# halajun/VDO_SLAM

Hardware: AMD Instinct MI355X
Metric: frames/sec (per-frame hot path, KITTI-0000-shaped 1242x375) + ms/LM-iter (batch factor graph) (higher is better)
Workload: dtype f64 (LM, RANSAC) / u8,i32,f32 (front-end, tracking)

## Files before the change

### __graft_entry__.py

```python
import os
import subprocess
import sys

ROOT = os.path.dirname(os.path.abspath(__file__))
if ROOT not in sys.path:
    sys.path.insert(0, ROOT)


def build() -> None:
    env = dict(os.environ)
    jobs = str(max(1, min(16, os.cpu_count() or 2)))
    subprocess.run(["make", "-C", os.path.join(ROOT, "vdo_slam_amd", "csrc"), "-j", jobs], check=True, env=env)
    subprocess.run(["make", "-C", os.path.join(ROOT, "vdo_slam_amd", "host")], check=True, env=env)
    subprocess.run(["make", "-C", os.path.join(ROOT, "oracle"), "-j", jobs], check=True, env=env)
    from tests import oracle_lib as _ol
    _ol.load_product_epnp()
    subprocess.run(["/opt/rocm/bin/hipcc", "--offload-arch=gfx950", "-O3", "-std=c++17", "-ffp-contract=off", "-Wno-unused-value",
                    os.path.join(ROOT, "tools", "lm_dev_check.hip"), "-o", os.path.join(ROOT, "tools", "lm_dev_check")], check=True, env=env)
    subprocess.run(["/opt/rocm/bin/hipcc", "--offload-arch=gfx950", "-O3", "-std=c++17", "-ffp-contract=off", "-munsafe-fp-atomics", "-Wno-unused-value",
                    os.path.join(ROOT, "tools", "dense_check.hip"), "-o", os.path.join(ROOT, "tools", "dense_check")], check=True, env=env)
    _ol.load_ref_orb()
    _ol.load_ref_track()
    _ol.load_ref_full()
    import vdo_slam_amd
    from vdo_slam_amd import _capi
    import ctypes
    lib = ctypes.CDLL(_capi.LIB_PATH)
    assert lib.vdo_version() >= 1


def smoke() -> None:
    import ctypes as C
    import numpy as np
    from vdo_slam_amd import _capi as K, synth
    from vdo_slam_amd.ba import BatchBA, Context
    from tests import oracle_lib

    g = synth.make_ba_graph(n_frames=10, n_static=400, n_objects=2, dyn_tracks_per_object=40, seed=7)
    ctx = Context(0)
    ba = BatchBA(ctx, g)
    ba.linearize()
    S = ba.system()
    o = oracle_lib.load()
    gc, keep = K.graph_to_c(g)
    R = K.BASystem(g)
    o.vdo_oracle_ba_linearize(C.byref(gc), C.byref(R.c))
    for name in ("Hpp", "bp", "Hll", "bl", "Hpl_eb", "Hll_et", "Hlp1_et", "Hlp2_et", "Hpp_ep"):
        a, b = getattr(S, name), getattr(R, name)
        scale = max(1e-300, np.abs(b).max())
        assert np.abs(a - b).max() <= 1e-10 * scale, f"smoke: block {name} differs from oracle"
    assert abs(S.robust_chi2 - R.robust_chi2) <= 1e-10 * abs(R.robust_chi2)
    st = ba.optimize(max_iterations=5, gain_threshold=1e-4)
    assert st.iterations >= 1 and st.final_chi2 <= st.initial_chi2
    from tests import frontend_ref as R2
    from tests.test_oracle_flow2 import run_oracle
    from vdo_slam_amd import synth_frames as SF
    from vdo_slam_amd.flow2 import Flow2Batch
    from vdo_slam_amd.frontend import ORBextractor
    prob = synth.make_flow2_problem(600, seed=3)
    b = Flow2Batch(ctx, [prob]); b.run(); r = b.fetch()[0]
    T_o, _, inl_o, ninl_o, st_o = run_oracle(o, prob)
    assert r["iterations"] == st_o.iterations and r["n_inliers"] == ninl_o and np.array_equal(r["inliers"], inl_o), "smoke: flow2 LM differs from oracle"
    assert np.abs(r["T"] - T_o).max() < 1e-8
    gray = SF.make_gray(11, 640, 200)
    kp = ORBextractor(ctx, 640, 200)(gray, descriptors=True)
    ref = R2.extract_desc(o, gray)
    assert np.array_equal(kp["x"], ref["x"]) and np.array_equal(kp["y"], ref["y"]) and np.array_equal(kp["octave"], ref["octave"]), "smoke: ORB keypoints differ from oracle"
    assert np.array_equal(kp["desc"], ref["desc"]), "smoke: rotated-BRIEF descriptor bits differ from oracle"
    ba.set_estimates(g.pose, g.point)
    st3 = ba.optimize(max_iterations=5, gain_threshold=1e-4, solver=3)
    assert (st3.iterations, st3.total_trials) == (st.iterations, st.total_trials) and abs(st3.final_chi2 - st.final_chi2) <= 1e-9 * st.final_chi2, "smoke: dense MFMA solve differs from PCG"
# ... 25 lines not shown
```

### vdo_slam_amd/csrc/flow2.hip

```cpp
#include <algorithm>
#include <cmath>
#include <cstdlib>
#include <cstring>
#include <type_traits>
#include <vector>

#include "../../include/vdo_slam_hip.h"
#include "ctx.hpp"
#include "lm_dev.hpp"

namespace vdo {

struct Flow2Dev {
  int n, max_iterations, ref_quirks, pad;
  int64_t off;
  int64_t out_off, out_total;
  double K[4], Twl[16], T0[16];
  double info_flow, info_prior, huber_delta, huber_dsqr, chi2_gate;
};

struct Flow2Arrays {
  const double* in;
  double* om;
  double *Xw, *f0, *f1, *err, *B2a, *B2b, *hla, *hlb, *bla, *blb, *xl;
// ... 64 lines not shown
  template <bool TRIAL> __device__ __forceinline__ void after_exchange(double hb) {
    const double h = tid > 0 ? s_h[tid - 1] : hb;
    if constexpr (TRIAL) hpt = h; else hpc = h;
  }
  __device__ __forceinline__ void accept() { fc0 = ft0; fc1 = ft1; cur = trial; hpc = hpt; }
};

struct F2MemStore {
  static constexpr bool kReg = false;
  const int N, first, c_lo, c_hi;
  double *obs, *meas, *Xw, *fcur, *ftry, *err, *xl;
  double *Bc, *Bt, *hc, *ht, *bc, *bt;
  template <class F> __device__ __forceinline__ void for_each(F&& f) { for (int i = first; i < c_hi; i += F2_THREADS) f(i); }
  __device__ __forceinline__ void set_point(int i, double o0, double o1, double m0, double m1, const double (&x)[3]) {
    obs[i] = o0; obs[N + i] = o1; meas[i] = m0; meas[N + i] = m1;
    Xw[i] = x[0]; Xw[N + i] = x[1]; Xw[2 * N + i] = x[2];
    fcur[i] = m0; fcur[N + i] = m1;
    xl[i] = 0.0; xl[N + i] = 0.0;
  }
  __device__ __forceinline__ void point(int i, double& o0, double& o1, double& m0, double& m1, double (&x)[3]) const {
    o0 = obs[i]; o1 = obs[N + i]; m0 = meas[i]; m1 = meas[N + i]; x[0] = Xw[i]; x[1] = Xw[N + i]; x[2] = Xw[2 * N + i];
  }
  __device__ __forceinline__ void flow_cur(int i, double& f0, double& f1) const { f0 = fcur[i]; f1 = fcur[N + i]; }
  __device__ __forceinline__ void set_flow_try(int i, double f0, double f1) { ftry[i] = f0; ftry[N + i] = f1; }
  __device__ __forceinline__ void get_xl(int i, double& x0, double& x1) const { x0 = xl[i]; x1 = xl[N + i]; }
  __device__ __forceinline__ void set_xl(int i, double x0, double x1) { xl[i] = x0; xl[N + i] = x1; }
  __device__ __forceinline__ void get_err(int i, double& e0, double& e1) const { e0 = err[i]; e1 = err[N + i]; }
  __device__ __forceinline__ void set_err(int i, double e0, double e1) { err[i] = e0; err[N + i] = e1; }
  __device__ __forceinline__ void lin_cur(int i, F2Lin& L) const {
#pragma unroll
    for (int a = 0; a < 12; ++a) L.B[a] = Bc[a * N + i];
    L.h = hc[i]; L.b0 = bc[i]; L.b1 = bc[N + i];
  }
  template <bool TRIAL> __device__ __forceinline__ void set_lin(int i, const F2Lin& L) {
    double* const B = TRIAL ? Bt : Bc; double* const h = TRIAL ? ht : hc; double* const b = TRIAL ? bt : bc;
#pragma unroll
    for (int a = 0; a < 12; ++a) B[a * N + i] = L.B[a];
    h[i] = L.h; b[i] = L.b0; b[N + i] = L.b1;
  }
  __device__ __forceinline__ double h_prev(int i, double hb) const { return i > c_lo ? hc[i - 1] : hb; }
  template <bool TRIAL> __device__ __forceinline__ void after_exchange(double) {}
  __device__ __forceinline__ void accept() {
    double* t_ = fcur; fcur = ftry; ftry = t_;
    t_ = Bc; Bc = Bt; Bt = t_; t_ = hc; hc = ht; ht = t_; t_ = bc; bc = bt; bt = t_;
  }
};

#ifdef F2_PROFILE
#define F2_TICK(slot) do { if (tid == 0) { const long long t_ = clock64(); s_prof[slot] += t_ - s_tprev; s_tprev = t_; } } while (0)
#else
#define F2_TICK(slot) do { } while (0)
#endif

__global__ __launch_bounds__(F2_THREADS) void k_flow2_lm(const Flow2Dev* __restrict__ probs, Flow2Arrays A) {
#ifdef F2_LINEAR_MAP
  const int prob = blockIdx.x / F2_CLUSTER, wg = blockIdx.x % F2_CLUSTER;
#else
  const int xcd = blockIdx.x & 7, rest = blockIdx.x >> 3;
  const int wg = rest % F2_CLUSTER, prob = (rest / F2_CLUSTER) * 8 + xcd;
#endif
  if (prob >= A.n_problems) return;
  const Flow2Dev P = probs[prob];
  const int N = P.n, tid = threadIdx.x;
  const int Gp = min(A.max_cluster, max(1, (N + F2_THREADS - 1) / F2_THREADS));
  if (wg >= Gp) return;
  __builtin_amdgcn_s_setprio(3);
  const int chunk = (N + Gp - 1) / Gp, c_lo = wg * chunk, c_hi = min(N, c_lo + chunk);
  const int first = c_lo + tid;
  Flow2Comm* comm = A.comm + prob;
  const int64_t off = P.off;
  const double* __restrict__ in_obs = A.in + 5 * off; const double* __restrict__ in_meas = in_obs + 2 * (size_t)N; const double* __restrict__ depth = in_obs + 4 * (size_t)N;
  vdo_flow2_result* res = (vdo_flow2_result*)A.out + prob;
  double* __restrict__ flow_out = (double*)(A.out + sizeof(vdo_flow2_result) * (size_t)A.n_problems) + 2 * P.out_off;
  unsigned char* __restrict__ inlier_out = (unsigned char*)((double*)(A.out + sizeof(vdo_flow2_result) * (size_t)A.n_problems) + 2 * P.out_total) + P.out_off;

  __shared__ double s_scr[F2_WAVES * 4], s_red[32];
  __shared__ double s_wpart[F2_WAVES * 32];
  __shared__ SE3d s_T, s_Ttry;
  __shared__ double s_Hc[27], s_xp[6], s_Hs[36], s_bs[6], s_xs[6];
  __shared__ double s_rho;
  __shared__ int s_ctrl[4];
  __shared__ double s_hlast;
  if (tid == 0) s_ctrl[3] = 0;
#ifdef F2_PROFILE
  __shared__ long long s_prof[16], s_tprev;
  if (tid == 0) { for (int i = 0; i < 16; ++i) s_prof[i] = 0; s_tprev = clock64(); }
#endif

  if (N < 3) {
    if (tid < 16) res->T[tid] = (tid % 5 == 0) ? 1.0 : 0.0;
    if (tid < N) { inlier_out[tid] = 0; flow_out[2 * tid] = in_meas[tid]; flow_out[2 * tid + 1] = in_meas[N + tid]; }
    if (tid == 0) { res->n_inliers = 0; res->iterations = 0; res->trials = 0; res->stop_reason = 0; res->initial_chi2 = res->final_chi2 = res->final_lambda = 0; }
    return;
  }
  const double fx = P.K[0], fy = P.K[1], cx = P.K[2], cy = P.K[3];
  const bool Q = P.ref_quirks != 0;
  if (tid < 6) s_xp[tid] = 0.0;
  if (tid == 0) {
    const double R[9] = {P.T0[0], P.T0[1], P.T0[2], P.T0[4], P.T0[5], P.T0[6], P.T0[8], P.T0[9], P.T0[10]};
    s_T.r = q_from_R(R);
    q_normalize_pos(s_T.r);
    s_T.t[0] = P.T0[3]; s_T.t[1] = P.T0[7]; s_T.t[2] = P.T0[11];
  }
  __syncthreads();

  int phase = 0;
  __shared__ double s_part[F2_CLUSTER][32];
  auto cluster_sum = [&](const int K, double& mx, double& hb) -> bool {
    if (Gp == 1) return true;
    const unsigned tag = A.tag_base + (unsigned)phase + 1u;
    if (tid < 31) {
      const double v = tid < K ? s_red[tid] : (tid == 29 ? mx : (tid == 30 ? hb : 0.0));
      const unsigned long long u = (unsigned long long)__double_as_longlong(v);
      const f2_u32x4 w = {(unsigned)u, tag, (unsigned)(u >> 32), tag};
      f2_slot_store(&comm->slot[phase & 1][wg][tid], w);
    }
    {
      const int g2 = tid >> 5, q = tid & 31;
      double v = 0.0;
      int bad = 0;
      if (g2 < Gp && q < 31) {
        const Flow2Slot* src = &comm->slot[phase & 1][g2][q];
        f2_u32x4 w = f2_slot_load(src);
        int spins = 0;
        while (w.y != tag || w.w != tag) {
          __builtin_amdgcn_s_sleep(1);
          if (++spins > (1 << 20)) { bad = 1; break; }
          w = f2_slot_load(src);
        }
        v = __longlong_as_double((long long)(((unsigned long long)w.z << 32) | (unsigned long long)w.x));
      }
      if (g2 < F2_CLUSTER) s_part[g2][q] = v;
      if (bad) s_ctrl[3] = 1;
    }
    __syncthreads();
    if (s_ctrl[3]) return false;
    if (tid < K) {
      double a = 0.0;
      for (int g2 = 0; g2 < Gp; ++g2) a += s_part[g2][tid];
      s_red[tid] = a;
    }
    if (tid == 32) {
      double m = 0.0;
      for (int g2 = 0; g2 < Gp; ++g2) m = fmax(m, s_part[g2][29]);
      s_red[31] = m;
      s_red[30] = wg > 0 ? s_part[wg - 1][30] : 0.0;
    }
    __syncthreads();
    mx = s_red[31]; hb = s_red[30];
    ++phase;
    return true;
  };
#define F2_CLUSTER_SUM(K, mx, hb) do { if (!cluster_sum(K, mx, hb)) { if (wg == 0 && tid == 0) { res->stop_reason = -1; res->iterations = -1; } return; } } while (0)

  auto dinv_q = [&](const double hh, const double lam, double& d0, double& d1, double& d2) {
    const double a0 = hh + lam;
    const double C00 = lam * lam, hl_ = hh * lam, al = a0 * lam;
    const double id = 1.0 / (C00 * a0);
    d0 = C00 * id; d1 = (-hl_) * id; d2 = al * id;
  };
  auto dinv_of = [&](const double hh, const double lam, double* Di) {
    const double a0 = hh + lam, a1 = 0.0, a2 = 0.0, a3 = hh + lam;
    const double id = 1.0 / (a0 * a3 - a1 * a2);
    Di[0] = a3 * id; Di[1] = -a1 * id; Di[2] = 0; Di[3] = -a2 * id; Di[4] = a0 * id; Di[5] = 0; Di[6] = 0; Di[7] = 0; Di[8] = 0;
  };

  auto solve_pose = [&](const double lambda, const int qmax, const double currentChi) __attribute__((always_inline)) {
    if (tid < 36) {
      const int a = tid / 6, c2 = tid - 6 * a;
      if (c2 <= a) {
        const int k = a * (a + 1) / 2 + c2;
        double v = s_Hc[k] - s_red[k];
        if (c2 == a) v += lambda;
        s_Hs[tid] = v;
      } else {
        s_Hs[tid] = s_Hc[c2 * (c2 + 1) / 2 + a];
      }
    } else if (tid < 42) {
      const int j = tid - 36;
      s_bs[j] = s_Hc[21 + j] - s_red[21 + j];
    }
    __syncthreads();
    F2_TICK(5);
    bool ok2w = false;
    if (tid < 64) ok2w = ldlt6_solve_lanes(s_Hs, s_bs, s_xs);
    if (tid == 0) {
      const bool ok2 = ok2w;
      F2_TICK(6);
      s_ctrl[2] = ok2 ? 1 : 0;
      if (ok2) {
#pragma unroll
        for (int j = 0; j < 6; ++j) s_xp[j] = s_xs[j];
      }
      double s = 0;
      for (int j = 0; j < 6; ++j) s += s_xp[j] * (lambda * s_xp[j] + s_Hc[21 + j]);
      s_rho = s;
      bool skip = false;
      if (!ok2 && qmax + 1 < 10) skip = (currentChi - 1.7976931348623157e308) / ((s + s_red[27]) + 1e-3) < 0;
      s_ctrl[1] = skip ? 1 : 0;
      if (!skip) s_Ttry = se3_exp_compose(s_xp, s_T);
      F2_TICK(7);
    }
    __syncthreads();
    F2_TICK(1);
  };

  auto lm_body = [&](auto& S) __attribute__((always_inline)) {
    constexpr bool kReg = std::remove_reference_t<decltype(S)>::kReg;
    S.for_each([&](const int i) {
      const double dz = depth[i];
      const double o0 = in_obs[i], o1 = in_obs[N + i], m0 = in_meas[i], m1 = in_meas[N + i];
      const double x = (o0 - cx) * dz / fx, y = (o1 - cy) * dz / fy;
      const double* W = P.Twl;
      const double xw[3] = {W[0] * x + W[1] * y + W[2] * dz + W[3], W[4] * x + W[5] * y + W[6] * dz + W[7], W[8] * x + W[9] * y + W[10] * dz + W[11]};
      S.set_point(i, o0, o1, m0, m1, xw);
    });

    auto sweep = [&](auto trial_c, const double lam, const bool ok2, const double hb_prev, const F2Pre& pre) -> double {
      constexpr bool TRIAL = decltype(trial_c)::value;
      const SE3d T = TRIAL ? s_Ttry : s_T;
      double xp[6];
#pragma unroll
      for (int j = 0; j < 6; ++j) xp[j] = s_xp[j];
      double acc[29];
#pragma unroll
      for (int k = 0; k < 29; ++k) acc[k] = 0.0;
      double hmax = 0.0;
      S.for_each([&](const int i) {
        double f0v, f1v;
        S.flow_cur(i, f0v, f1v);
        if (TRIAL) {
          const bool hp = kReg || (Q && i == pre.i);
          F2Lin L;
          if (!kReg && hp) {
#pragma unroll
            for (int a = 0; a < 12; ++a) L.B[a] = pre.B[a];
            L.b0 = pre.b0; L.b1 = pre.b1;
          } else {
            S.lin_cur(i, L);
          }
          const double b0 = L.b0, b1 = L.b1;
          double t0 = 0, t1 = 0;
#pragma unroll
          for (int a = 0; a < 6; ++a) { t0 += L.B[2 * a] * (-xp[a]); t1 += L.B[2 * a + 1] * (-xp[a]); }
          const double c0 = b0 + t0, c1 = b1 + t1;
          double x0, x1;
          if (Q) {
            double d0, d1, d2, p2_ = 0;
            if (hp) { d0 = pre.d0; d1 = pre.d1; d2 = pre.d2; p2_ = pre.p2; }
            else if constexpr (!kReg) {
              dinv_q(L.h, lam, d0, d1, d2);
              if (i > 0) { double p0_, p1_; dinv_q(S.h_prev(i, hb_prev), lam, p0_, p1_, p2_); }
            }
// ... 174 lines not shown
          lambda *= fmax(lower, alpha); ni = 2; currentChi = tempChi; built = true;
          S.accept();
          hb_cur = hb_try;
          if (tid < 27) s_Hc[tid] = s_red[tid];
          if (tid == 32) s_T = s_Ttry;
        } else {
          lambda *= ni; ni *= 2; built = false;
        }
        __syncthreads();
        F2_TICK(3);
        ++qmax; ++total_trials;
      } while (rho < 0 && qmax < 10);
      int result;
      if (qmax == 10 || rho == 0) result = 1;
      else {
        if ((iniChi - currentChi) * 1e3 < iniChi) nBad++; else nBad = 0;
        result = nBad >= 3 ? 1 : 0;
      }
      ok = (result == 0);
      if (!ok) stop_reason = 1;
      if (chi2_check < last_err_chi && it > 0) { ok = false; stop_reason = 2; }
      chi2_check = last_err_chi;
    }
    double cnt[1] = {0.0};
    const float gate = (float)P.chi2_gate;
    S.for_each([&](const int i) {
      double e0, e1, f0, f1;
      S.get_err(i, e0, e1);
      S.flow_cur(i, f0, f1);
      const float chi2 = (float)(e0 * (P.info_flow * e0) + e1 * (P.info_flow * e1));
      const bool outl = chi2 > gate;
      inlier_out[i] = outl ? 0 : 1;
      cnt[0] += outl ? 0.0 : 1.0;
      flow_out[2 * i] = f0;
      flow_out[2 * i + 1] = f1;
    });
    block_reduce<1>(cnt, s_scr, s_red);
    { double d_ = 0, e_ = 0; F2_CLUSTER_SUM(1, d_, e_); }
    if (tid == 0 && wg == 0) {
      se3_to_matrix(s_T, res->T);
      res->n_inliers = (int)(s_red[0] + 0.5);
      res->iterations = it; res->trials = total_trials; res->stop_reason = stop_reason;
      res->initial_chi2 = initial_chi2; res->final_chi2 = last_err_chi; res->final_lambda = lambda;
#ifdef F2_PROFILE
      for (int k = 0; k < 14; ++k) res->T[k] = (double)s_prof[k];
#endif
    }
#ifdef F2_PROFILE
    __syncthreads();
    if (tid == 0 && wg < 2) res->T[14 + wg] = (double)(__builtin_amdgcn_s_getreg((4 - 1) << 11 | 0 << 6 | 20) & 0xf) + 100.0 * blockIdx.x;
#endif
  };

  const bool REG = chunk <= F2_THREADS && !A.force_general;
  if (REG) {
    __shared__ double s_h[F2_THREADS];
    F2RegStore S{first, tid, first < c_hi, s_h};
    lm_body(S);
  } else {
    double* const om = A.om + 4 * off;
    F2MemStore S{N, first, c_lo, c_hi, om, om + 2 * (size_t)N, A.Xw + 3 * off, A.f0 + 2 * off, A.f1 + 2 * off, A.err + 2 * off, A.xl + 2 * off,
                 A.B2a + 12 * off, A.B2b + 12 * off, A.hla + off, A.hlb + off, A.bla + 2 * off, A.blb + 2 * off};
    lm_body(S);
  }
}

}

using namespace vdo;

struct vdo_flow2_batch {
  vdo_ctx* ctx = nullptr;
  int n_problems = 0;
  int64_t total = 0;
  std::vector<void*> allocs;
  Flow2Dev* d_probs = nullptr;
  Flow2Arrays A{};
  std::vector<int64_t> offs;
  std::vector<int> ns;
  char* h_pin = nullptr;
  double* h_up = nullptr;
  std::vector<Flow2Dev> hp;
  std::vector<int> caps;
  bool probs_dirty = false;
  unsigned run_seq = 0;
  const Flow2Dev* d_probs_run = nullptr;
};

extern "C" int vdo_flow2_batch_destroy(vdo_flow2_batch* b) {
  if (!b) return VDO_OK;
  if (b->ctx) { ctx_bind(b->ctx); hipStreamSynchronize(b->ctx->stream); }
  for (void* p : b->allocs) hipFree(p);
  if (b->h_pin) hipHostFree(b->h_pin);
  if (b->h_up) hipHostFree(b->h_up);
  delete b;
  return VDO_OK;
}

static void fill_descriptor(Flow2Dev& d, const vdo_flow2_problem& p) {
  d.max_iterations = p.max_iterations; d.ref_quirks = p.ref_quirks;
  std::memcpy(d.K, p.K, sizeof(d.K)); std::memcpy(d.Twl, p.Twl, sizeof(d.Twl)); std::memcpy(d.T0, p.T0, sizeof(d.T0));
  d.info_flow = p.info_flow; d.info_prior = p.info_prior; d.huber_delta = p.huber_delta;
  d.huber_dsqr = (double)(float)(p.huber_delta * p.huber_delta);
  d.chi2_gate = p.chi2_gate;
}

static void pack_planes(double* st, const vdo_flow2_problem& p) {
  const size_t n = (size_t)p.n;
  double *po = st, *pm = st + 2 * n;
  for (size_t i = 0; i < n; ++i) { po[i] = p.obs[2 * i]; po[n + i] = p.obs[2 * i + 1]; pm[i] = p.flow[2 * i]; pm[n + i] = p.flow[2 * i + 1]; }
  std::memcpy(st + 4 * n, p.depth, sizeof(double) * n);
}
// ... 70 lines not shown
  if (rc != VDO_OK) return rc;
  vdo_flow2_batch* b = *out;
  if (hipHostMalloc((void**)&b->h_up, sizeof(double) * 5 * (size_t)std::max<int64_t>(tot, 1) + sizeof(Flow2Dev) * (size_t)n_problems, hipHostMallocMapped) != hipSuccess) { b->h_up = nullptr; vdo_flow2_batch_destroy(b); return set_error(VDO_ERR_OOM, "hipHostMalloc failed"); }
  void* dp = nullptr;
  if (hipHostGetDevicePointer(&dp, b->h_up, 0) != hipSuccess || !dp) { vdo_flow2_batch_destroy(b); return set_error(VDO_ERR_NO_DEVICE, "hipHostGetDevicePointer failed"); }
  b->A.in = (const double*)dp;
  b->d_probs_run = (const Flow2Dev*)((const double*)dp + 5 * (size_t)std::max<int64_t>(tot, 1));
  for (int k = 0; k < n_problems; ++k) { b->hp[k].n = 0; b->ns[k] = 0; }
  std::memcpy(b->h_up + 5 * (size_t)std::max<int64_t>(tot, 1), b->hp.data(), sizeof(Flow2Dev) * (size_t)n_problems);
  if (hipStreamSynchronize(ctx->stream) != hipSuccess) { vdo_flow2_batch_destroy(b); return set_error(VDO_ERR_NO_DEVICE, "flow2 reserve failed"); }
  return VDO_OK;
}

extern "C" int vdo_flow2_batch_set(vdo_flow2_batch* b, int k, const vdo_flow2_problem* p) {
  if (!b || k < 0 || k >= b->n_problems || !b->h_up) return set_error(VDO_ERR_INVALID, "vdo_flow2_batch_set: bad argument / batch not created by vdo_flow2_batch_reserve");
  int rc = ctx_bind(b->ctx);
  if (rc != VDO_OK) return rc;
  Flow2Dev& d = b->hp[k];
  const int n = p ? p->n : 0;
  if (n < 0 || n > b->caps[k] || (n > 0 && (!p->obs || !p->flow || !p->depth))) return set_error(VDO_ERR_INVALID, "vdo_flow2_batch_set: %d points do not fit slot %d (capacity %d)", n, k, b->caps[k]);
  if (n) {
    pack_planes(b->h_up + 5 * b->offs[k], *p);
    fill_descriptor(d, *p);
  }
  d.n = n; b->ns[k] = n;
  b->probs_dirty = true;
  return VDO_OK;
}

extern "C" int vdo_flow2_batch_run(vdo_flow2_batch* b) {
  if (!b) return set_error(VDO_ERR_INVALID, "null handle");
  int rc = ctx_bind(b->ctx);
  if (rc != VDO_OK) return rc;
  if (b->probs_dirty) {
    int64_t used = 0;
    for (int k = 0; k < b->n_problems; ++k) { b->hp[k].out_off = used; used += b->hp[k].n; }
    for (int k = 0; k < b->n_problems; ++k) b->hp[k].out_total = used;
    std::memcpy(b->h_up + 5 * (size_t)std::max<int64_t>(b->total, 1), b->hp.data(), sizeof(Flow2Dev) * (size_t)b->n_problems);
    b->probs_dirty = false;
  }
  b->A.tag_base = (++b->run_seq) << 16;
  {
    int budget = 256;
    if (const char* e = std::getenv("VDO_LM_CLUSTER_BUDGET")) budget = std::max(1, std::atoi(e));
    int mc = F2_CLUSTER;
    for (; mc > 1; mc >>= 1) {
      int64_t wgs = 0;
      for (int k = 0; k < b->n_problems; ++k) if (b->ns[k] >= 3) wgs += std::min(mc, std::max(1, (b->ns[k] + F2_THREADS - 1) / F2_THREADS));
      if (wgs <= budget) break;
    }
    b->A.max_cluster = mc;
  }
  { const char* e = std::getenv("VDO_LM_GENERAL"); b->A.force_general = (e && std::atoi(e) != 0) ? 1 : 0; }
  hipLaunchKernelGGL(k_flow2_lm, dim3(((b->n_problems + 7) / 8) * 8 * F2_CLUSTER), dim3(F2_THREADS), 0, b->ctx->stream, b->d_probs_run ? b->d_probs_run : (const Flow2Dev*)b->d_probs, b->A);
  hipError_t e = hipGetLastError();
  if (e != hipSuccess) return set_error(VDO_ERR_NO_DEVICE, "k_flow2_lm launch: %s", hipGetErrorString(e));
  return VDO_OK;
}

extern "C" int vdo_flow2_batch_fetch(vdo_flow2_batch* b, vdo_flow2_result* results, double** flow_out, uint8_t** inlier_out) {
  if (!b || !results) return set_error(VDO_ERR_INVALID, "null argument");
  int rc = ctx_bind(b->ctx);
  if (rc != VDO_OK) return rc;
  const size_t NP = (size_t)b->n_problems;
  size_t used = 0;
  for (int k = 0; k < b->n_problems; ++k) used += (size_t)b->ns[k];
  hipError_t e = hipStreamSynchronize(b->ctx->stream);
  if (e != hipSuccess) return set_error(VDO_ERR_NO_DEVICE, "flow2 fetch: %s", hipGetErrorString(e));
  const vdo_flow2_result* pr = (const vdo_flow2_result*)b->h_pin;
  const double* pf = (const double*)(b->h_pin + sizeof(vdo_flow2_result) * NP);
  const uint8_t* pi = (const uint8_t*)(pf + 2 * used);
  std::memcpy(results, pr, sizeof(vdo_flow2_result) * NP);
  for (size_t k = 0; k < NP; ++k) if (pr[k].iterations < 0) return set_error(VDO_ERR_NO_DEVICE, "k_flow2_lm: the workgroup cluster of problem %d lost its barrier", (int)k);
  size_t o = 0;
  for (int k = 0; k < b->n_problems; ++k) {
    const size_t n = (size_t)b->ns[k];
    if (n && flow_out && flow_out[k]) std::memcpy(flow_out[k], pf + 2 * o, sizeof(double) * 2 * n);
    if (n && inlier_out && inlier_out[k]) std::memcpy(inlier_out[k], pi + o, n);
    o += n;
  }
  return VDO_OK;
}

extern "C" int vdo_flow2_optimize(vdo_ctx* ctx, const vdo_flow2_problem* p, vdo_flow2_result* result, double* flow_out, uint8_t* inlier_out) {
  vdo_flow2_batch* b = nullptr;
  int rc = vdo_flow2_batch_create(ctx, 1, p, &b);
  if (rc != VDO_OK) return rc;
  rc = vdo_flow2_batch_run(b);
  if (rc == VDO_OK) rc = vdo_flow2_batch_fetch(b, result, &flow_out, &inlier_out);
  vdo_flow2_batch_destroy(b);
  return rc;
}
```

### vdo_slam_amd/csrc/lm_dev.hpp

```cpp
#pragma once
#include <hip/hip_runtime.h>

#ifndef F2_THREADS
#define F2_THREADS 256
#endif
#define F2_WAVES (F2_THREADS / 64)

namespace vdo {

struct Q4 { double x, y, z, w; };
struct SE3d { Q4 r; double t[3]; };

__device__ __forceinline__ void q_rotate(const Q4& q, const double* v, double* o) {
  double ux = q.y * v[2] - q.z * v[1], uy = q.z * v[0] - q.x * v[2], uz = q.x * v[1] - q.y * v[0];
  ux += ux; uy += uy; uz += uz;
  o[0] = v[0] + q.w * ux + (q.y * uz - q.z * uy);
  o[1] = v[1] + q.w * uy + (q.z * ux - q.x * uz);
  o[2] = v[2] + q.w * uz + (q.x * uy - q.y * ux);
}
template <int I>
__device__ __forceinline__ Q4 q_from_R_neg_trace(const double* m) {
  constexpr int J = (I + 1) % 3, K = (J + 1) % 3;
  double t = sqrt(m[4 * I] - m[4 * J] - m[4 * K] + 1.0);
  double c[3];
// ... 160 lines not shown
      double temp[6];
#pragma unroll
      for (int j = 0; j < k; ++j) temp[j] = VDO_M(j, j) * VDO_M(k, j);
      double s = 0;
#pragma unroll
      for (int j = 0; j < k; ++j) s += VDO_M(k, j) * temp[j];
      VDO_M(k, k) -= s;
#pragma unroll
      for (int i = k + 1; i < 6; ++i) {
        double t = 0;
#pragma unroll
        for (int j = 0; j < k; ++j) t += VDO_M(i, j) * temp[j];
        VDO_M(i, k) -= t;
      }
    }
    const double akk = VDO_M(k, k);
    const bool valid = fabs(akk) > 0.0;
    if (k == 0 && !valid) { sign = 0; zero = true; continue; }
    if (valid) {
#pragma unroll
      for (int i = k + 1; i < 6; ++i) VDO_M(i, k) /= akk;
    }
    if (sign == 1) { if (akk < 0) sign = 2; }
    else if (sign == -1) { if (akk > 0) sign = 2; }
    else if (sign == 0) { if (akk > 0) sign = 1; else if (akk < 0) sign = -1; }
  }
  if (!(sign == 1 || sign == 0)) return false;
  double y[6];
#pragma unroll
  for (int k = 0; k < 6; ++k) y[k] = b[ord[k]];
#pragma unroll
  for (int i = 0; i < 6; ++i) {
#pragma unroll
    for (int j = 0; j < i; ++j) y[i] -= VDO_M(i, j) * y[j];
  }
#pragma unroll
  for (int i = 0; i < 6; ++i) { if (fabs(VDO_M(i, i)) > 2.2250738585072014e-308) y[i] /= VDO_M(i, i); else y[i] = 0; }
#pragma unroll
  for (int i = 5; i >= 0; --i) {
#pragma unroll
    for (int j = i + 1; j < 6; ++j) y[i] -= VDO_M(j, i) * y[j];
  }
#undef VDO_M
#pragma unroll
  for (int k = 0; k < 6; ++k) x[ord[k]] = y[k];
  return true;
}

__device__ __forceinline__ double readlane_f64(double v, const int lane) {
  const unsigned long long u = (unsigned long long)__double_as_longlong(v);
  const unsigned lo = (unsigned)__builtin_amdgcn_readlane((int)(unsigned)u, lane), hi = (unsigned)__builtin_amdgcn_readlane((int)(unsigned)(u >> 32), lane);
  return __longlong_as_double((long long)(((unsigned long long)hi << 32) | lo));
}
__device__ __forceinline__ bool ldlt6_solve_lanes(const double* A, const double* b, double* x) {
  const int lane = threadIdx.x & 63;
  const int li = lane < 6 ? lane : 5;
  int ord[6];
  {
    double dd[6];
#pragma unroll
    for (int i = 0; i < 6; ++i) dd[i] = fabs(A[7 * i]);
    const double dm = fabs(A[7 * li]);
    int rank = 0, ties = 0;
#pragma unroll
    for (int j = 0; j < 6; ++j) { rank += dd[j] > dm ? 1 : 0; ties += (dd[j] == dm && j != li) ? 1 : 0; }
    bool simple = __ballot(lane < 6 && ties != 0) == 0ull;
#pragma unroll
    for (int q = 0; q < 6; ++q) {
      const unsigned long long mk = __ballot(lane < 6 && rank == q);
      simple = simple && mk != 0ull;
      ord[q] = (int)__builtin_ctzll(mk | (1ull << 63));
    }
    if (!simple) {
#pragma unroll
      for (int i = 0; i < 6; ++i) ord[i] = i;
#pragma unroll
      for (int k = 0; k < 5; ++k) {
        int big = k;
        double bv = dd[k];
#pragma unroll
        for (int i = k + 1; i < 6; ++i) if (dd[i] > bv) { bv = dd[i]; big = i; }
#pragma unroll
        for (int bb = k + 1; bb < 6; ++bb)
          if (big == bb) { const double t = dd[k]; dd[k] = dd[bb]; dd[bb] = t; const int u = ord[k]; ord[k] = ord[bb]; ord[bb] = u; }
      }
    }
  }
  int r = ord[0];
#pragma unroll
  for (int i = 1; i < 6; ++i) r = li == i ? ord[i] : r;
  double m[6];
#pragma unroll
  for (int j = 0; j < 6; ++j) { const int c = ord[j]; m[j] = r >= c ? A[r * 6 + c] : A[c * 6 + r]; }
  double y = b[r];
  const double a00 = readlane_f64(m[0], 0);
  if (!(fabs(a00) > 0.0)) {
    bool ok = false;
    if (lane == 0) ok = ldlt6_solve_perm(A, b, x);
    return __builtin_amdgcn_readfirstlane((int)ok) != 0;
  }
  double D[6];
  double dself = 0.0;
  bool neg = false;
#pragma unroll
  for (int k = 0; k < 6; ++k) {
    if (k > 0) {
      double temp[6];
#pragma unroll
      for (int j = 0; j < k; ++j) temp[j] = D[j] * readlane_f64(m[j], k);
      double t = 0;
#pragma unroll
      for (int j = 0; j < k; ++j) t += m[j] * temp[j];
      m[k] -= t;
    }
    const double akk = readlane_f64(m[k], k);
    D[k] = akk;
    dself = lane == k ? akk : dself;
    const bool valid = fabs(akk) > 0.0;
    const double q = m[k] / akk;
    m[k] = (valid && lane > k) ? q : m[k];
    neg = neg || akk < 0;
  }
  if (neg) return false;
#pragma unroll
  for (int j = 0; j < 5; ++j) { const double yj = readlane_f64(y, j); const double u = y - m[j] * yj; y = lane > j ? u : y; }
  y = fabs(dself) > 2.2250738585072014e-308 ? y / dself : 0.0;
  double yf[6];
  yf[5] = readlane_f64(y, 5);
#pragma unroll
  for (int i = 4; i >= 0; --i) {
    double yi = readlane_f64(y, i);
#pragma unroll
    for (int j = i + 1; j < 6; ++j) yi -= readlane_f64(m[i], j) * yf[j];
    yf[i] = yi;
  }
  double mine = yf[0];
#pragma unroll
  for (int i = 1; i < 6; ++i) mine = li == i ? yf[i] : mine;
  if (lane < 6) x[r] = mine;
  return true;
}

__device__ __forceinline__ void inv3_dev(const double* a, double* o) {
  const double C00 = a[4] * a[8] - a[5] * a[7];
  const double C10 = a[2] * a[7] - a[1] * a[8];
  const double C20 = a[1] * a[5] - a[2] * a[4];
  const double det = (C00 * a[0] + C10 * a[3]) + C20 * a[6];
  const double id = 1.0 / det;
  o[0] = C00 * id; o[1] = C10 * id; o[2] = C20 * id;
  o[3] = (a[5] * a[6] - a[3] * a[8]) * id; o[4] = (a[0] * a[8] - a[2] * a[6]) * id; o[5] = (a[2] * a[3] - a[0] * a[5]) * id;
  o[6] = (a[3] * a[7] - a[4] * a[6]) * id; o[7] = (a[1] * a[6] - a[0] * a[7]) * id; o[8] = (a[0] * a[4] - a[1] * a[3]) * id;
}

__device__ __forceinline__ void huber_f2(double e, double delta, double dsqr, double& r0, double& r1) {
  if (e <= dsqr) { r0 = e; r1 = 1.0; }
  else { const double s = sqrt(e); r0 = 2 * s * delta - dsqr; r1 = delta / s; }
}

template <int K>
__device__ __forceinline__ void block_reduce(double (&v)[K], double* scratch, double* out) {
  const int lane = threadIdx.x & 63, wv = threadIdx.x >> 6;
#pragma unroll
  for (int i = 0; i < K; ++i) {
    double t = v[i];
#pragma unroll
    for (int off = 32; off > 0; off >>= 1) t += __shfl_down(t, off, 64);
    if (lane == 0) scratch[wv * K + i] = t;
  }
  __syncthreads();
  if (threadIdx.x < K) {
    double a = 0.0;
#pragma unroll
    for (int w = 0; w < F2_WAVES; w += 4)
      a += (scratch[w * K + threadIdx.x] + scratch[(w + 1) * K + threadIdx.x]) + (scratch[(w + 2) * K + threadIdx.x] + scratch[(w + 3) * K + threadIdx.x]);
    out[threadIdx.x] = a;
  }
  __syncthreads();
}

template <int K>
__device__ __forceinline__ void block_reduce_wide(const double (&v)[K], double* wide, double* out) {
  static_assert(K * 8 <= F2_THREADS, "one 8-lane group per quantity");
  constexpr int LD = F2_THREADS + 1;
  const int tid = threadIdx.x;
#pragma unroll
  for (int i = 0; i < K; ++i) wide[i * LD + tid] = v[i];
  __syncthreads();
  const int q = tid >> 3, part = tid & 7;
  double a = 0.0;
  if (q < K) {
    const double* col = wide + q * LD + part;
#pragma unroll 8
    for (int j = 0; j < F2_THREADS / 8; ++j) a += col[8 * j];
  }
  a += __shfl_down(a, 4, 8);
  a += __shfl_down(a, 2, 8);
  a += __shfl_down(a, 1, 8);
  if (q < K && part == 0) out[q] = a;
  __syncthreads();
}

template <int CTRL>
__device__ __forceinline__ double dpp_f64(double v) {
  const long long u = __double_as_longlong(v);
  const int lo = __builtin_amdgcn_update_dpp(0, (int)(unsigned)u, CTRL, 0xF, 0xF, false);
  const int hi = __builtin_amdgcn_update_dpp(0, (int)(unsigned)((unsigned long long)u >> 32), CTRL, 0xF, 0xF, false);
  return __longlong_as_double((long long)(((unsigned long long)(unsigned)hi << 32) | (unsigned long long)(unsigned)lo));
}
template <bool ROW32>
__device__ __forceinline__ void rows_swap_f64(double& a, double& b) {
  const unsigned long long ua = (unsigned long long)__double_as_longlong(a), ub = (unsigned long long)__double_as_longlong(b);
  const auto lo = ROW32 ? __builtin_amdgcn_permlane32_swap((unsigned)ua, (unsigned)ub, false, false) : __builtin_amdgcn_permlane16_swap((unsigned)ua, (unsigned)ub, false, false);
  const auto hi = ROW32 ? __builtin_amdgcn_permlane32_swap((unsigned)(ua >> 32), (unsigned)(ub >> 32), false, false)
                        : __builtin_amdgcn_permlane16_swap((unsigned)(ua >> 32), (unsigned)(ub >> 32), false, false);
  a = __longlong_as_double((long long)(((unsigned long long)hi[0] << 32) | lo[0]));
  b = __longlong_as_double((long long)(((unsigned long long)hi[1] << 32) | lo[1]));
}
__device__ __forceinline__ int bfly_quantity(int lane) { return ((lane >> 5) << 4) | (((lane >> 4) & 1) << 3) | (((lane >> 3) & 1) << 2) | (((lane >> 2) & 1) << 1) | ((lane >> 1) & 1); }
template <int K>
__device__ __forceinline__ double wave_reduce32(const double (&acc)[K]) {
  static_assert(K <= 32, "at most 32 quantities");
  const int lane = threadIdx.x & 63;
  double v[32];
#pragma unroll
  for (int i = 0; i < 32; ++i) v[i] = i < K ? acc[i] : 0.0;
#pragma unroll
  for (int j = 0; j < 16; ++j) { rows_swap_f64<true>(v[j], v[j + 16]); v[j] = v[j] + v[j + 16]; }
#pragma unroll
  for (int j = 0; j < 8; ++j) { rows_swap_f64<false>(v[j], v[j + 8]); v[j] = v[j] + v[j + 8]; }
  {
    const bool up = (lane & 8) != 0;
#pragma unroll
    for (int j = 0; j < 4; ++j) { const double keep = up ? v[j + 4] : v[j], send = up ? v[j] : v[j + 4]; v[j] = keep + dpp_f64<0x128>(send); }
  }
  {
    const bool up = (lane & 4) != 0;
#pragma unroll
    for (int j = 0; j < 2; ++j) { const double keep = up ? v[j + 2] : v[j], send = up ? v[j] : v[j + 2]; v[j] = keep + dpp_f64<0x141>(send); }
  }
  {
    const bool up = (lane & 2) != 0;
    const double keep = up ? v[1] : v[0], send = up ? v[0] : v[1];
    v[0] = keep + dpp_f64<0x4E>(send);
  }
  return v[0] + dpp_f64<0xB1>(v[0]);
}
template <int K>
__device__ __forceinline__ void block_reduce_bfly(const double (&acc)[K], double* part, double* out) {
  const int lane = threadIdx.x & 63, wv = threadIdx.x >> 6;
  const double t = wave_reduce32<K>(acc);
  if ((lane & 1) == 0) part[wv * 32 + bfly_quantity(lane)] = t;
  __syncthreads();
  if (threadIdx.x < K) {
    double a = part[threadIdx.x];
#pragma unroll
    for (int w = 1; w < F2_WAVES; ++w) a += part[w * 32 + threadIdx.x];
    out[threadIdx.x] = a;
  }
  __syncthreads();
}

__device__ inline void se3_to_matrix(const SE3d& S, double* T) {
  const Q4 q = S.r;
  const double tx = 2 * q.x, ty = 2 * q.y, tz = 2 * q.z;
  const double twx = tx * q.w, twy = ty * q.w, twz = tz * q.w, txx = tx * q.x, txy = ty * q.x, txz = tz * q.x, tyy = ty * q.y, tyz = tz * q.y, tzz = tz * q.z;
  T[0] = 1 - (tyy + tzz); T[1] = txy - twz; T[2] = txz + twy; T[3] = S.t[0];
  T[4] = txy + twz; T[5] = 1 - (txx + tzz); T[6] = tyz - twx; T[7] = S.t[1];
  T[8] = txz - twy; T[9] = tyz + twx; T[10] = 1 - (txx + tyy); T[11] = S.t[2];
  T[12] = 0; T[13] = 0; T[14] = 0; T[15] = 1;
}
// ... 3 lines not shown
```

Measured before the change: 1376.

## Fuse pose solve staging into wave-parallel LDLT and lane-parallel SE3 compose

The 6x6 pose solve now reads the reduced Hessian directly from the packed accumulators inside the lane-parallel LDLT, which removes a staging pass and a block barrier. The SE3 exponential-and-compose step is spread across the first wave's lanes with DPP shuffles instead of running on a single thread. The LM kernel is also templated on register vs memory storage, and the host launches a specialized instance so the unused path is compiled out. The aim is a shorter serial critical path per LM iteration; the cost is more complex lane-level code whose floating-point results must stay bit-identical to the oracle.

```diff
diff --git a/__graft_entry__.py b/__graft_entry__.py
--- a/__graft_entry__.py
+++ b/__graft_entry__.py
@@ -17,6 +17,8 @@
     _ol.load_product_epnp()
     subprocess.run(["/opt/rocm/bin/hipcc", "--offload-arch=gfx950", "-O3", "-std=c++17", "-ffp-contract=off", "-Wno-unused-value",
                     os.path.join(ROOT, "tools", "lm_dev_check.hip"), "-o", os.path.join(ROOT, "tools", "lm_dev_check")], check=True, env=env)
+    subprocess.run(["/opt/rocm/bin/hipcc", "--offload-arch=gfx950", "-O3", "-std=c++17", "-ffp-contract=off", "-Wno-unused-value",
+                    os.path.join(ROOT, "tools", "lm_serial_check.hip"), "-o", os.path.join(ROOT, "tools", "lm_serial_check")], check=True, env=env)
     subprocess.run(["/opt/rocm/bin/hipcc", "--offload-arch=gfx950", "-O3", "-std=c++17", "-ffp-contract=off", "-munsafe-fp-atomics", "-Wno-unused-value",
                     os.path.join(ROOT, "tools", "dense_check.hip"), "-o", os.path.join(ROOT, "tools", "dense_check")], check=True, env=env)
     _ol.load_ref_orb()
diff --git a/vdo_slam_amd/csrc/flow2.hip b/vdo_slam_amd/csrc/flow2.hip
--- a/vdo_slam_amd/csrc/flow2.hip
+++ b/vdo_slam_amd/csrc/flow2.hip
@@ -140,6 +140,8 @@
 #define F2_TICK(slot) do { } while (0)
 #endif
 
+enum { F2_STORE_BOTH = 0, F2_STORE_REG = 1, F2_STORE_MEM = 2 };
+template <int STORE>
 __global__ __launch_bounds__(F2_THREADS) void k_flow2_lm(const Flow2Dev* __restrict__ probs, Flow2Arrays A) {
 #ifdef F2_LINEAR_MAP
   const int prob = blockIdx.x / F2_CLUSTER, wg = blockIdx.x % F2_CLUSTER;
@@ -165,7 +167,7 @@
   __shared__ double s_scr[F2_WAVES * 4], s_red[32];
   __shared__ double s_wpart[F2_WAVES * 32];
   __shared__ SE3d s_T, s_Ttry;
-  __shared__ double s_Hc[27], s_xp[6], s_Hs[36], s_bs[6], s_xs[6];
+  __shared__ double s_Hc[27], s_xp[6], s_Hs[36], s_bs[6];
   __shared__ double s_rho;
   __shared__ int s_ctrl[4];
   __shared__ double s_hlast;
@@ -254,39 +256,20 @@
   };
 
   auto solve_pose = [&](const double lambda, const int qmax, const double currentChi) __attribute__((always_inline)) {
-    if (tid < 36) {
-      const int a = tid / 6, c2 = tid - 6 * a;
-      if (c2 <= a) {
-        const int k = a * (a + 1) / 2 + c2;
-        double v = s_Hc[k] - s_red[k];
-        if (c2 == a) v += lambda;
-        s_Hs[tid] = v;
-      } else {
-        s_Hs[tid] = s_Hc[c2 * (c2 + 1) / 2 + a];
-      }
-    } else if (tid < 42) {
-      const int j = tid - 36;
-      s_bs[j] = s_Hc[21 + j] - s_red[21 + j];
-    }
-    __syncthreads();
-    F2_TICK(5);
-    bool ok2w = false;
-    if (tid < 64) ok2w = ldlt6_solve_lanes(s_Hs, s_bs, s_xs);
-    if (tid == 0) {
-      const bool ok2 = ok2w;
+    if (tid < 64) {
+      double xu[6];
+      const bool ok2 = ldlt6_solve_lanes_reduced(s_Hc, s_red, lambda, s_Hs, s_bs, s_xp, xu, [&]() { F2_TICK(5); });
       F2_TICK(6);
-      s_ctrl[2] = ok2 ? 1 : 0;
-      if (ok2) {
-#pragma unroll
-        for (int j = 0; j < 6; ++j) s_xp[j] = s_xs[j];
+      if (!ok2) {
+#pragma unroll
+        for (int j = 0; j < 6; ++j) xu[j] = s_xp[j];
       }
       double s = 0;
-      for (int j = 0; j < 6; ++j) s += s_xp[j] * (lambda * s_xp[j] + s_Hc[21 + j]);
-      s_rho = s;
+      for (int j = 0; j < 6; ++j) s += xu[j] * (lambda * xu[j] + s_Hc[21 + j]);
       bool skip = false;
       if (!ok2 && qmax + 1 < 10) skip = (currentChi - 1.7976931348623157e308) / ((s + s_red[27]) + 1e-3) < 0;
-      s_ctrl[1] = skip ? 1 : 0;
-      if (!skip) s_Ttry = se3_exp_compose(s_xp, s_T);
+      if (tid == 0) { s_ctrl[2] = ok2 ? 1 : 0; s_rho = s; s_ctrl[1] = skip ? 1 : 0; }
+      if (!skip) se3_exp_compose_lanes(xu, &s_T, &s_Ttry, s_Hs);
       F2_TICK(7);
     }
     __syncthreads();
@@ -567,12 +550,22 @@
 #endif
   };
 
-  const bool REG = chunk <= F2_THREADS && !A.force_general;
-  if (REG) {
-    __shared__ double s_h[F2_THREADS];
-    F2RegStore S{first, tid, first < c_hi, s_h};
-    lm_body(S);
-  } else {
+  const bool REG = STORE == F2_STORE_REG || (STORE == F2_STORE_BOTH && chunk <= F2_THREADS && !A.force_general);
+  if constexpr (STORE == F2_STORE_REG) {
+    if (chunk > F2_THREADS) {
+      if (wg == 0 && tid == 0) { res->stop_reason = -1; res->iterations = -1; }
+      return;
+    }
+  }
+  if constexpr (STORE != F2_STORE_MEM) {
+    if (REG) {
+      __shared__ double s_h[F2_THREADS];
+      F2RegStore S{first, tid, first < c_hi, s_h};
+      lm_body(S);
+      return;
+    }
+  }
+  if constexpr (STORE != F2_STORE_REG) {
     double* const om = A.om + 4 * off;
     F2MemStore S{N, first, c_lo, c_hi, om, om + 2 * (size_t)N, A.Xw + 3 * off, A.f0 + 2 * off, A.f1 + 2 * off, A.err + 2 * off, A.xl + 2 * off,
                  A.B2a + 12 * off, A.B2b + 12 * off, A.hla + off, A.hlb + off, A.bla + 2 * off, A.blb + 2 * off};
@@ -749,7 +742,21 @@
     b->A.max_cluster = mc;
   }
   { const char* e = std::getenv("VDO_LM_GENERAL"); b->A.force_general = (e && std::atoi(e) != 0) ? 1 : 0; }
-  hipLaunchKernelGGL(k_flow2_lm, dim3(((b->n_problems + 7) / 8) * 8 * F2_CLUSTER), dim3(F2_THREADS), 0, b->ctx->stream, b->d_probs_run ? b->d_probs_run : (const Flow2Dev*)b->d_probs, b->A);
+  bool any_reg = false, any_mem = false;
+  for (int k = 0; k < b->n_problems; ++k) {
+    const int n = b->ns[k];
+    if (n < 3) continue;
+    const int gp = std::min(b->A.max_cluster, std::max(1, (n + F2_THREADS - 1) / F2_THREADS));
+    if ((n + gp - 1) / gp <= F2_THREADS && !b->A.force_general) any_reg = true; else any_mem = true;
+  }
+  const dim3 grid(((b->n_problems + 7) / 8) * 8 * F2_CLUSTER), block(F2_THREADS);
+  const Flow2Dev* probs = b->d_probs_run ? b->d_probs_run : (const Flow2Dev*)b->d_probs;
+#ifdef F2_SINGLE_KERNEL
+  any_reg = any_mem = true;
+#endif
+  if (!any_mem) hipLaunchKernelGGL(k_flow2_lm<F2_STORE_REG>, grid, block, 0, b->ctx->stream, probs, b->A);
+  else if (!any_reg) hipLaunchKernelGGL(k_flow2_lm<F2_STORE_MEM>, grid, block, 0, b->ctx->stream, probs, b->A);
+  else hipLaunchKernelGGL(k_flow2_lm<F2_STORE_BOTH>, grid, block, 0, b->ctx->stream, probs, b->A);
   hipError_t e = hipGetLastError();
   if (e != hipSuccess) return set_error(VDO_ERR_NO_DEVICE, "k_flow2_lm launch: %s", hipGetErrorString(e));
   return VDO_OK;
diff --git a/vdo_slam_amd/csrc/lm_dev.hpp b/vdo_slam_amd/csrc/lm_dev.hpp
--- a/vdo_slam_amd/csrc/lm_dev.hpp
+++ b/vdo_slam_amd/csrc/lm_dev.hpp
@@ -236,15 +236,21 @@
   const unsigned lo = (unsigned)__builtin_amdgcn_readlane((int)(unsigned)u, lane), hi = (unsigned)__builtin_amdgcn_readlane((int)(unsigned)(u >> 32), lane);
   return __longlong_as_double((long long)(((unsigned long long)hi << 32) | lo));
 }
-__device__ __forceinline__ bool ldlt6_solve_lanes(const double* A, const double* b, double* x) {
+__device__ __forceinline__ void wave_lds_sync() {
+  __builtin_amdgcn_fence(__ATOMIC_RELEASE, "wavefront");
+  __builtin_amdgcn_wave_barrier();
+  __builtin_amdgcn_fence(__ATOMIC_ACQUIRE, "wavefront");
+}
+template <bool XU, class GetA, class GetB, class Rare, class Gathered>
+__device__ __forceinline__ bool ldlt6_lanes_core(GetA&& get, GetB&& rhs, Rare&& rare, Gathered&& gathered, double* x, double (&xu)[6]) {
   const int lane = threadIdx.x & 63;
   const int li = lane < 6 ? lane : 5;
   int ord[6];
   {
+    const double dm = fabs(get(li, li));
     double dd[6];
 #pragma unroll
-    for (int i = 0; i < 6; ++i) dd[i] = fabs(A[7 * i]);
-    const double dm = fabs(A[7 * li]);
+    for (int i = 0; i < 6; ++i) dd[i] = readlane_f64(dm, i);
     int rank = 0, ties = 0;
 #pragma unroll
     for (int j = 0; j < 6; ++j) { rank += dd[j] > dm ? 1 : 0; ties += (dd[j] == dm && j != li) ? 1 : 0; }
@@ -275,14 +281,11 @@
   for (int i = 1; i < 6; ++i) r = li == i ? ord[i] : r;
   double m[6];
 #pragma unroll
-  for (int j = 0; j < 6; ++j) { const int c = ord[j]; m[j] = r >= c ? A[r * 6 + c] : A[c * 6 + r]; }
-  double y = b[r];
+  for (int j = 0; j < 6; ++j) { const int c = ord[j]; m[j] = get(max(r, c), min(r, c)); }
+  double y = rhs(r);
+  gathered();
   const double a00 = readlane_f64(m[0], 0);
-  if (!(fabs(a00) > 0.0)) {
-    bool ok = false;
-    if (lane == 0) ok = ldlt6_solve_perm(A, b, x);
-    return __builtin_amdgcn_readfirstlane((int)ok) != 0;
-  }
+  if (!(fabs(a00) > 0.0)) return rare();
   double D[6];
   double dself = 0.0;
   bool neg = false;
@@ -322,7 +325,53 @@
 #pragma unroll
   for (int i = 1; i < 6; ++i) mine = li == i ? yf[i] : mine;
   if (lane < 6) x[r] = mine;
+  if constexpr (XU) {
+#pragma unroll
+    for (int j = 0; j < 6; ++j) xu[j] = readlane_f64(mine, (int)__builtin_ctzll(__ballot(lane < 6 && r == j) | (1ull << 63)));
+  }
   return true;
+}
+__device__ __forceinline__ bool ldlt6_solve_lanes(const double* A, const double* b, double* x) {
+  double unused[6];
+  return ldlt6_lanes_core<false>([&](const int r, const int c) { return A[r * 6 + c]; }, [&](const int r) { return b[r]; },
+                          [&]() {
+                            bool ok = false;
+                            if ((threadIdx.x & 63) == 0) ok = ldlt6_solve_perm(A, b, x);
+                            return __builtin_amdgcn_readfirstlane((int)ok) != 0;
+                          },
+                          []() {}, x, unused);
+}
+template <class Gathered>
+__device__ __forceinline__ bool ldlt6_solve_lanes_reduced(const double* Hc, const double* red, const double lambda, double* A_scr, double* b_scr,
+                                                          double* x, double (&xu)[6], Gathered&& gathered) {
+  const int lane = threadIdx.x & 63;
+  auto get = [&](const int r, const int c) {
+    const int k = ((r * (r + 1)) >> 1) + c;
+    const double v = Hc[k] - red[k], vl = v + lambda;
+    return c == r ? vl : v;
+  };
+  auto rhs = [&](const int r) { return Hc[21 + r] - red[21 + r]; };
+  bool staged = false;
+  auto rare = [&]() {
+    if (lane < 36) {
+      const int a = lane / 6, c2 = lane - 6 * a;
+      A_scr[lane] = c2 <= a ? get(a, c2) : Hc[c2 * (c2 + 1) / 2 + a];
+    } else if (lane < 42) {
+      b_scr[lane - 36] = rhs(lane - 36);
+    }
+    wave_lds_sync();
+    bool ok = false;
+    if (lane == 0) ok = ldlt6_solve_perm(A_scr, b_scr, x);
+    wave_lds_sync();
+    staged = true;
+    return __builtin_amdgcn_readfirstlane((int)ok) != 0;
+  };
+  const bool ok = ldlt6_lanes_core<true>(get, rhs, rare, gathered, x, xu);
+  if (staged && ok) {
+#pragma unroll
+    for (int j = 0; j < 6; ++j) xu[j] = x[j];
+  }
+  return ok;
 }
 
 __device__ __forceinline__ void inv3_dev(const double* a, double* o) {
@@ -400,6 +449,76 @@
   a = __longlong_as_double((long long)(((unsigned long long)hi[0] << 32) | lo[0]));
   b = __longlong_as_double((long long)(((unsigned long long)hi[1] << 32) | lo[1]));
 }
+__device__ __forceinline__ void se3_exp_compose_lanes(const double (&u)[6], const SE3d* Tp, SE3d* out, double* tab) {
+  const int lane = threadIdx.x & 63;
+  const int p = lane & 3, qd = (lane >> 2) & 3;
+  const int r = p < 3 ? p : 0, c = qd < 3 ? qd : 0;
+  const int i1 = r == 2 ? 0 : r + 1, i2 = r == 0 ? 2 : r - 1;
+  const double* Tq = &Tp->r.x;
+  const double b0 = Tq[p], b1 = Tq[p < 3 ? 3 : 0], b2 = Tq[p == 0 ? 2 : (p == 1 ? 0 : 1)], b3 = Tq[p == 0 ? 1 : (p == 1 ? 2 : (p == 2 ? 0 : 2))];
+  const double v0 = Tp->t[r], v1 = Tp->t[i1], v2 = Tp->t[i2];
+  const double ox = u[0], oy = u[1], oz = u[2], u3 = u[3], u4 = u[4], u5 = u[5];
+  double om;
+  {
+    const int k = 3 - r - c;
+    const double w_ = k == 0 ? ox : (k == 1 ? oy : oz);
+    const bool neg = (c - r + 3) % 3 == 1;
+    om = r == c ? 0.0 : (neg ? -w_ : w_);
+    if (lane < 12 && p < 3) tab[3 * r + c] = om;
+  }
+  const double theta = sqrt(ox * ox + oy * oy + oz * oz);
+  const bool tiny = theta < 0.00001;
+  double a = 0, b = 0, c_ = 0;
+  if (!tiny) {
+    double sn, cs;
+    if (theta < 0.3) sincos_small(theta, sn, cs); else { sn = sin(theta); cs = cos(theta); }
+    a = sn / theta; b = (1 - cs) / (theta * theta); c_ = (theta - sn) / cube_rn(theta);
+  }
+  wave_lds_sync();
+  const double om2 = tab[3 * r] * tab[c] + tab[3 * r + 1] * tab[3 + c] + tab[3 * r + 2] * tab[6 + c];
+  const double id = r == c ? 1.0 : 0.0;
+  double R, V;
+  if (tiny) {
+    R = id + om + om2;
+    V = R;
+  } else {
+    R = (id + a * om) + b * om2;
+    V = (id + b * om) + c_ * om2;
+  }
+  const double pe = V * (c == 0 ? u3 : (c == 1 ? u4 : u5));
+  const double Et = (pe + dpp_f64<0x104>(pe)) + dpp_f64<0x108>(pe);
+  double Ru[9];
+#pragma unroll
+  for (int i = 0; i < 3; ++i) {
+#pragma unroll
+    for (int j = 0; j < 3; ++j) Ru[3 * i + j] = readlane_f64(R, 4 * j + i);
+  }
+  Q4 e = q_from_R(Ru);
+  if (e.w < 0) { e.x = -e.x; e.y = -e.y; e.z = -e.z; e.w = -e.w; }
+  const double en = sqrt(e.x * e.x + e.y * e.y + e.z * e.z + e.w * e.w);
+  double ec = p == 0 ? e.x : (p == 1 ? e.y : (p == 2 ? e.z : e.w));
+  ec /= en;
+  const double ew = dpp_f64<0xFF>(ec);
+  const double e1 = dpp_f64<0xC9>(ec), e2 = dpp_f64<0xD2>(ec);
+  double uu = e1 * v2 - e2 * v1;
+  uu += uu;
+  const double uu1 = dpp_f64<0xC9>(uu), uu2 = dpp_f64<0xD2>(uu);
+  const double rt = v0 + ew * uu + (e1 * uu2 - e2 * uu1);
+  const double ot = Et + rt;
+  const double t0 = ew * b0;
+  double t1 = dpp_f64<0x24>(ec) * b1;
+  double t2 = dpp_f64<0x49>(ec) * b2;
+  const double t3 = dpp_f64<0x92>(ec) * b3;
+  if (p == 3) { t1 = -t1; t2 = -t2; }
+  double oc = t0 + t1 + t2 - t3;
+  if (dpp_f64<0xFF>(oc) < 0) oc = -oc;
+  const double sq = oc * oc;
+  const double on = sqrt(dpp_f64<0x00>(sq) + dpp_f64<0x55>(sq) + dpp_f64<0xAA>(sq) + dpp_f64<0xFF>(sq));
+  oc /= on;
+  if (lane < 4) (&out->r.x)[lane] = oc;
+  if (lane < 3) out->t[lane] = ot;
+}
+
 __device__ __forceinline__ int bfly_quantity(int lane) { return ((lane >> 5) << 4) | (((lane >> 4) & 1) << 3) | (((lane >> 3) & 1) << 2) | (((lane >> 2) & 1) << 1) | ((lane >> 1) & 1); }
 template <int K>
 __device__ __forceinline__ double wave_reduce32(const double (&acc)[K]) {
```

After: 1308. -5.0%, worse.
